# ChristophReich1996/Multi-StyleGAN

Measured on AMD Instinct MI355X. Metric: training images/sec (G+D step, 256^2, seq=3x2ch), higher is better.
Workload: dtype bf16

## Files before the change

### include/msg_hip.h

```cpp
#ifndef MSG_HIP_H
#define MSG_HIP_H

#ifdef __cplusplus
extern "C" {
#endif

enum { MSG_OK = 0, MSG_EINVAL = -1, MSG_EUNSUPPORTED = -2, MSG_ELAUNCH = -3 };
enum { MSG_F32 = 0, MSG_BF16 = 1, MSG_F16 = 2, MSG_F64 = 3, MSG_F32_SPLIT = 4 };

#define MSG_ABI_VERSION 5
int msg_abi_version(void);
const char* msg_build_arch(void);
const char* msg_strerror(int code);

int msg_upfirdn2d(const void* x, const float* fir, void* y, int dtype,
                  int major, int in_h, int in_w, int minor, int kh, int kw,
                  int up_x, int up_y, int down_x, int down_y,
                  int pad_x0, int pad_x1, int pad_y0, int pad_y1, void* stream);

int msg_upfirdn2d_pitched(const void* x, const float* fir, void* y, int dtype,
                          int major, int in_h, int in_w, int minor, int in_pitch, int kh, int kw,
                          int up_x, int up_y, int down_x, int down_y,
                          int pad_x0, int pad_x1, int pad_y0, int pad_y1, void* stream);

// ... 128 lines not shown
                         int B, int IH, int IW, int Cx, int Ck, int OH, int OW, int N, int ldy,
                         int kh, int kw, int stride, int pad, long long w_batch_stride,
                         const float* act_bias, const float* noise, const float* noise_weight,
                         int noise_batch, float alpha, float scale, void* stream);
int msg_conv2d_fprop_act_mask(const void* x, const void* w, void* y, int dtype,
                              int B, int IH, int IW, int Cx, int Ck, int OH, int OW, int N, int ldy,
                              int kh, int kw, int stride, int pad, long long w_batch_stride,
                              const float* act_bias, const float* noise, const float* noise_weight,
                              int noise_batch, float alpha, float scale, unsigned char* mask, void* stream);

int msg_conv2d_fprop_residual(const void* x, const void* w, void* y, int dtype,
                              int B, int IH, int IW, int Cx, int Ck, int OH, int OW, int N, int ldy,
                              int kh, int kw, int stride, int pad, long long w_batch_stride,
                              const void* residual, int res_ld, float gain, void* stream);

long long msg_conv2d_fprop_act_backward_workspace(int dtype, int B, int IH, int IW, int Cx, int Ck, int OH, int OW,
                                                  int N, int kh, int kw, long long w_batch_stride, int has_noise);
int msg_conv2d_fprop_act_backward(const void* x, const void* w, void* y, int dtype,
                                  int B, int IH, int IW, int Cx, int Ck, int OH, int OW, int N, int ldy,
                                  int kh, int kw, int stride, int pad, long long w_batch_stride,
                                  const void* residual, int res_ld,
                                  const unsigned char* sign_mask, int mask_tile_m, int mask_tile_n,
                                  const void* sign_map, int sign_ld, float alpha, float scale,
                                  float* grad_bias, const float* noise, int noise_batch, float* grad_noise_weight,
                                  float* ws, long long ws_floats, void* stream);

int msg_act_pointwise_head(const void* x, const float* bias, const float* w, float* y, int dtype,
                           long long npix, int C, float wscale, float alpha, float scale, void* stream);
long long msg_act_pointwise_head_backward_workspace(long long npix, int C);
int msg_act_pointwise_head_backward(const void* x, const float* bias, const float* w, const float* gy, void* gx,
// ... 43 lines not shown
```

### multi_stylegan_amd/conv_ops.py

```python
import math
import os
from typing import Optional, Tuple

import torch
from torch.autograd import Function

from . import _lib
from ._autograd import _derive


def _vec(dtype) -> int:
    return 8 if dtype == torch.bfloat16 else 4


def _round_up(n: int, m: int) -> int:
    return (n + m - 1) // m * m


def _padded_nhwc(b, c, h, w, dtype, device):
    cx = _round_up(c, _vec(dtype))
    buf = torch.empty((b, h, w, cx), dtype=dtype, device=device)
    if cx != c:
        buf[..., c:].zero_()
    return buf.permute(0, 3, 1, 2)[:, :c]
# ... 323 lines not shown
    def set(mode: str) -> None:
        fp32_contraction(mode).__enter__()


def _contraction_code(t: torch.Tensor, mode: Optional[str] = None) -> int:
    code = _lib.dtype_code(t)
    mode = FP32_CONTRACTION if mode is None else mode
    return _SPLIT_CODES[mode] if (code == _lib.MSG_F32 and mode != "exact") else code


_PLANS = {_lib.MSG_PLAN_REG: ("conv_fprop_reg", None), _lib.MSG_PLAN_DMA: ("conv_fprop_dma", None),
          _lib.MSG_PLAN_PP: ("conv_fprop_pp", None), _lib.MSG_PLAN_ROW3: ("conv_fprop_row3", 256),
          _lib.MSG_PLAN_ROW3N: ("conv_fprop_row3n", 128), _lib.MSG_PLAN_THIN: ("conv_fprop_thin", None)}
_PLAN_CACHE: dict = {}
_WGRAD_WS_CACHE: dict = {}


def _launch_fprop(x, wk, ck, bias, n, out_hw, kh, kw, stride, pad, in_up, pixel_shuffle, per_sample, c_real,
                  flops=None, act=None, residual=None, out=None, mode=None):
    dev = _lib.require_gpu(x, wk, bias)
    xv, cx = _nhwc_view(x)
    b, _, ih, iw = xv.shape
    oh, ow = out_hw
    if out is not None:
        y, ldy = _nhwc_view(out)
        if y is not out or pixel_shuffle or out.shape != (b, n, oh, ow) or out.dtype != x.dtype or n % _vec(x.dtype):
            raise _lib.MsgHipError(f"conv fprop: destination {tuple(out.shape)} / {out.stride()} for a {(b, n, oh, ow)} result")
    elif pixel_shuffle:
        y, ldy = _alloc_out(b, n // 4, 2 * oh, 2 * ow, x.dtype, dev)
    else:
# ... 8 lines not shown
        raise _lib.MsgHipError(f"conv fprop: weight image {tuple(wk.shape)} smaller than {n} x {kh * kw} x {ck}")
    wstride = wk.stride(0) if per_sample else 0
    if flops is None:
        flops = 2.0 * b * oh * ow * n * kh * kw * c_real / (in_up * in_up)
    key = "conv_fprop"
    if _lib.kernel_clock.enabled:
        plan = _lib.lib().msg_conv2d_fprop_plan(_lib.dtype_code(x), b, ih, iw, cx, ck, oh, ow, n, kh, kw, wstride)
        key = _PLANS[_lib.MSG_PLAN_REG if plan == _lib.MSG_PLAN_THIN and act is not None else plan][0]
        if x.dtype == torch.bfloat16 and bias is None and act is None and residual is None and \
                _lib.lib().msg_conv2d_fprop_upconv_eligible(b, ih, iw, cx, ck, oh, ow, n, kh, kw, stride, pad, in_up,
                                                           int(pixel_shuffle), wstride):
            key = "conv_fprop_upconv"
        if _CLOCK_SHAPES:
            key += f"|B{b} {ih}x{iw}->{oh}x{ow} {c_real}->{n} {kh}x{kw} s{stride} up{in_up}" \
                   f"{' ps' if pixel_shuffle else ''}{' per-sample' if per_sample else ''}|"
    with _lib.on_device(dev), _lib.kernel_clock.span((key, 'bf16' if x.dtype == torch.bfloat16 else 'f32'), flops):
        if residual is not None:
            assert bias is None and act is None and in_up == 1 and not pixel_shuffle
            rv, res_ld = _nhwc_view(residual[0])
            assert rv.shape == (b, n, oh, ow) and rv.dtype == x.dtype
            code = _lib.lib().msg_conv2d_fprop_residual(
                xv.data_ptr(), wk.data_ptr(), y.data_ptr(), _contraction_code(x, mode), b, ih, iw, cx, ck, oh, ow, n, ldy, kh, kw,
                stride, pad, wstride, rv.data_ptr(), res_ld, float(residual[1]), _lib.stream_of(dev))
        elif act is None:
            code = _lib.lib().msg_conv2d_fprop(
                xv.data_ptr(), wk.data_ptr(), _lib.ptr(bias), y.data_ptr(), _contraction_code(x, mode), b, ih, iw, cx, ck, oh,
                ow, n, ldy, kh, kw, stride, pad, in_up, int(pixel_shuffle), wstride, _lib.stream_of(dev))
        else:
            assert bias is None and in_up == 1 and not pixel_shuffle
            act_bias, noise, noise_w, alpha, scale = act[:5]
            _lib.require_gpu(x, act_bias, noise, noise_w)
            mask = None
            if len(act) > 5 and act[5] is not None and kh == 3 and stride == 1 and pad == 1:
                pkey = (x.dtype, b, ih, iw, cx, ck, oh, ow, n, kh, kw, wstride)
                mplan = _PLAN_CACHE.get(pkey)
                if mplan is None:
                    mplan = _PLAN_CACHE[pkey] = _lib.lib().msg_conv2d_fprop_plan(_lib.dtype_code(x), b, ih, iw, cx, ck, oh, ow,
                                                                                n, kh, kw, wstride)
                tile = _PLANS[mplan][1]
                if tile:
                    from .op_static.fused_act import sign_mask_for
                    mask = sign_mask_for(b, n, oh, ow, x.dtype, dev)
# ... 1320 lines not shown
```

### multi_stylegan_amd/csrc/conv_dispatch.h

```cpp
#pragma once
#include "msg_common.h"

struct ConvProblem {
    int dtype;
    int split;
    int B, IH, IW, Cx, Ck, OH, OW, N, ldy;
    int kh, kw, stride, pad, in_up, pixel_shuffle;
    long long w_batch_stride;

    bool per_sample() const { return w_batch_stride != 0; }
    int samples() const { return per_sample() ? B : 1; }
    long long mtot() const { return per_sample() ? (long long)OH * OW : (long long)B * OH * OW; }
    int esz() const { return dtype == MSG_BF16 ? 2 : 4; }
    long long x_bstride() const { return (long long)IH * IW * Cx; }
    long long y_bstride() const { return (pixel_shuffle ? 4ll : 1ll) * OH * OW * ldy; }
    long long x_bytes() const { return (long long)(per_sample() ? 1 : B) * IH * IW * Cx * esz(); }
    long long w_bytes() const { return (long long)N * kh * kw * Ck * esz(); }
    bool fits31() const { return x_bytes() < 0x7ffffff0ll && w_bytes() < 0x7ffffff0ll; }
};

enum ConvKernel {
    CONV_THIN_N, CONV_THIN_K,
    CONV_UPCONV,
    CONV_ROW3, CONV_ROW3N,
    CONV_PP,
    CONV_DMA, CONV_REG, CONV_REG_LEAN, CONV_REG_SPLIT
};

struct ConvPlan {
    ConvKernel kernel;
    int tile_m, tile_n;
    bool supported;
};

inline int conv_act_mode(const ActEpilogue* act) { return act ? act->enabled : 0; }

template <typename P>
inline void conv_fill_common(P& p, const ConvProblem& q, const ActEpilogue* act) {
    p.B = q.B; p.IH = q.IH; p.IW = q.IW; p.Cx = q.Cx; p.Ck = q.Ck; p.OH = q.OH; p.OW = q.OW; p.N = q.N; p.ldy = q.ldy;
    p.per_sample = q.per_sample();
    if (act) p.act = *act;
    p.x_bstride = q.x_bstride();
    p.w_bstride = q.w_batch_stride;
    p.y_bstride = q.y_bstride();
    p.Mtot = (int)q.mtot();
}
template <typename P>
// ... 32 lines not shown
```

### multi_stylegan_amd/csrc/conv_fprop.hip

```cpp
#include "conv_dispatch.h"
#include <stdlib.h>

typedef __bf16 bf16v8 __attribute__((ext_vector_type(8)));
typedef const __attribute__((address_space(1))) char* gptr_t;
typedef const __attribute__((address_space(1))) u32x4* gvec_t;
typedef __attribute__((address_space(3))) char* lds_t;

struct ConvParams {
    int B, IH, IW, Cx, Ck, OH, OW, N, ldy;
    int kh, kw, stride, pad, in_up, pixel_shuffle, per_sample;
    long long x_bstride, w_bstride, y_bstride;
    int Mtot, n_chunks, n_iters, m_tiles, n_tiles;
    ActEpilogue act;
};

constexpr int BM = 128, BN = 128, ROWB = 128;
constexpr int STAGE_BYTES = (BM + BN) * ROWB;
__device__ __attribute__((aligned(256))) unsigned int g_zero_page[16384];

__device__ __forceinline__ int swz(int row, int slot) { return row * ROWB + ((slot ^ ((row >> 1) & 7)) << 4); }

template <int SPLIT>
__device__ __forceinline__ void split_park(const u32x4& raw, char* dst) {
    uint2 pl[3];
#pragma unroll
    for (int h = 0; h < 2; ++h) {
        const float x0 = __uint_as_float(raw[2 * h]), x1 = __uint_as_float(raw[2 * h + 1]);
        const unsigned hp = (unsigned)f2bf(x0) | ((unsigned)f2bf(x1) << 16);
        const float r0 = x0 - __uint_as_float(hp << 16), r1 = x1 - __uint_as_float(hp & 0xffff0000u);
        const unsigned mp = (unsigned)f2bf(r0) | ((unsigned)f2bf(r1) << 16);
        (h ? pl[0].y : pl[0].x) = hp;
        (h ? pl[1].y : pl[1].x) = mp;
        if constexpr (SPLIT == 3) {
            const float q0 = r0 - __uint_as_float(mp << 16), q1 = r1 - __uint_as_float(mp & 0xffff0000u);
            (h ? pl[2].y : pl[2].x) = (unsigned)f2bf(q0) | ((unsigned)f2bf(q1) << 16);
        }
    }
#pragma unroll
    for (int p = 0; p < SPLIT; ++p) *reinterpret_cast<uint2*>(dst + p * 64) = pl[p];
}

template <typename T, bool DMA, int LEAN = 0, int SPLIT = 0>
__global__ __launch_bounds__(256, LEAN ? LEAN : 2) void conv_fprop_kernel(const T* __restrict__ x, const T* __restrict__ w,
                                                            T* __restrict__ y, const float* __restrict__ bias,
                                                            ConvParams p) {
    constexpr int VEC = 16 / sizeof(T);
    constexpr int BKE = ROWB / sizeof(T);
    static_assert(!LEAN || (!DMA && sizeof(T) == 2), "lean variant: bf16, register staging");
    static_assert(SPLIT == 0 || sizeof(T) == 4, "split-bf16 products are a mode of the fp32-storage kernel");
    static_assert(SPLIT == 0 || !DMA, "the split planes are written from the staging registers");
    constexpr int SROW = SPLIT ? SPLIT * 64 + 16 : ROWB;
    constexpr int STAGE = SPLIT ? (BM + BN) * SROW : STAGE_BYTES;
    constexpr bool ONE_STAGE = LEAN != 0 || SPLIT == 3;
    constexpr int SMEM_BYTES = ONE_STAGE ? (STAGE > 65536 || sizeof(T) == 2 ? STAGE : 65536) : 2 * STAGE;
    __shared__ __attribute__((aligned(16))) char smem[SMEM_BYTES];

    const int tid = threadIdx.x, lane = tid & 63, wid = tid >> 6;
    const int wm = wid >> 1, wn = wid & 1;
    const int lr = lane & 31, lh = lane >> 5;
    const unsigned L = xcd_remap(blockIdx.x, gridDim.x);
    const int n0 = (int)(L % p.n_tiles) * BN;
    const int m0 = (int)(L / p.n_tiles) * BM;
    const int bz = blockIdx.z;

    const int wid_u = __builtin_amdgcn_readfirstlane(wid);
    const int slot_phys = tid & 7;
    int row_of[4];
#pragma unroll
    for (int j = 0; j < 4; ++j) row_of[j] = DMA ? (wid * 32 + 8 * j + (lane >> 3)) : ((tid >> 3) + 32 * j);
    const int slot = DMA ? 0 : slot_phys;
    int a_ih0[4], a_iw0[4];
    long long a_boff[4];
    int a_slot[4];
    bool a_ok[4];
    const int ohw = p.OH * p.OW;
#pragma unroll
    for (int j = 0; j < 4; ++j) {
        const int m = m0 + row_of[j];
// ... 9 lines not shown
                     ((long long)a_ih0[j] * p.IW + a_iw0[j]) * p.Cx) * (long long)sizeof(T);
        a_slot[j] = slot_j;
    }
    const int taps = p.kh * p.kw;
    const gptr_t xbase = (gptr_t)x;
    const gptr_t zbase = (gptr_t)g_zero_page;
    const long long zoff = slot_phys * 16;
    gptr_t pa[4];
    gptr_t pb[4];
    {
        const gptr_t wb = (gptr_t)w + (p.per_sample ? (long long)bz * p.w_bstride : 0) * (long long)sizeof(T);
#pragma unroll
        for (int j = 0; j < 4; ++j) {
            const int n = n0 + row_of[j];
            const bool ok = n < p.N;
            pb[j] = (ok ? wb : zbase) + (ok ? ((long long)n * taps * p.Ck + a_slot[j] * VEC) * (long long)sizeof(T) : zoff);
            pa[j] = zbase;
        }
    }
    msg_desc_t d_x = {0, 0, 0, 0}, d_w = {0, 0, 0, 0};
    unsigned lds0 = 0;
    int va[4] = {MSG_DMA_OOB, MSG_DMA_OOB, MSG_DMA_OOB, MSG_DMA_OOB}, vb[4] = {MSG_DMA_OOB, MSG_DMA_OOB, MSG_DMA_OOB, MSG_DMA_OOB};
    if constexpr (DMA) {
        d_x = msg_make_desc((const char*)x + (p.per_sample ? (long long)bz * p.x_bstride * (long long)sizeof(T) : 0));
        d_w = msg_make_desc((const char*)w + (p.per_sample ? (long long)bz * p.w_bstride * (long long)sizeof(T) : 0));
        lds0 = (unsigned)(unsigned long long)(lds_t)smem;
#pragma unroll
        for (int j = 0; j < 4; ++j) {
            const int n = n0 + row_of[j];
            vb[j] = n < p.N ? (int)(((long long)n * taps * p.Ck + a_slot[j] * VEC) * (long long)sizeof(T)) : MSG_DMA_OOB;
        }
    }
    const bool ragged = (p.Cx % BKE) != 0;
    int ld_tap = -1, ld_chunk = p.n_chunks - 1;
    int kh_ = 0, kw_ = -1;
    int st_off[4];
#pragma unroll
    for (int j = 0; j < 4; ++j) st_off[j] = swz(row_of[j], a_slot[j]);

    f32x16 acc[2][2];
#pragma unroll
    for (int i = 0; i < 2; ++i)
#pragma unroll
        for (int j = 0; j < 2; ++j)
#pragma unroll
            for (int e = 0; e < 16; ++e) acc[i][j][e] = 0.f;

    u32x4 ra[4], rb[4];
    int dma_stage = 0;
    auto load_next = [&]() __attribute__((always_inline)) {
        if (++ld_chunk == p.n_chunks) {
            ld_chunk = 0;
            ++ld_tap;
            if (++kw_ == p.kw) { kw_ = 0; ++kh_; }
            if (p.in_up == 1) {
                const long long tap_off = ((long long)kh_ * p.IW + kw_) * p.Cx * (long long)sizeof(T);
#pragma unroll
                for (int j = 0; j < 4; ++j) {
                    const bool ok = a_ok[j] & ((unsigned)(a_ih0[j] + kh_) < (unsigned)p.IH) &
                                    ((unsigned)(a_iw0[j] + kw_) < (unsigned)p.IW);
                    pa[j] = (ok ? xbase : zbase) + (ok ? a_boff[j] + tap_off : zoff);
                    if constexpr (DMA) va[j] = ok ? (int)(a_boff[j] + tap_off) : MSG_DMA_OOB;
                }
            } else {
#pragma unroll
                for (int j = 0; j < 4; ++j) {
                    const int ih = a_ih0[j] + kh_, iw = a_iw0[j] + kw_;
                    bool ok = a_ok[j] & (ih >= 0) & (iw >= 0) & (ih % p.in_up == 0) & (iw % p.in_up == 0);
                    const int ihs = ih / p.in_up, iws = iw / p.in_up;
                    ok = ok & (ihs < p.IH) & (iws < p.IW);
                    const long long off = a_boff[j] + ((long long)(ihs - a_ih0[j]) * p.IW + (iws - a_iw0[j])) * p.Cx * (long long)sizeof(T);
                    pa[j] = (ok ? xbase : zbase) + (ok ? off : zoff);
                    if constexpr (DMA) va[j] = ok ? (int)off : MSG_DMA_OOB;
                }
            }
        }
#pragma unroll
        for (int j = 0; j < 4; ++j) {
            const bool c_bad = ragged && (ld_chunk * BKE + a_slot[j] * VEC + VEC > p.Cx);
            gptr_t a_addr = pa[j];
            if (c_bad) a_addr = zbase + zoff;
            if constexpr (DMA) {
                const unsigned la = lds0 + dma_stage * STAGE + (wid_u * 32 + 8 * j) * ROWB;
                msg_dma16(d_x, la, c_bad ? MSG_DMA_OOB : va[j], ld_chunk * ROWB);
                msg_dma16(d_w, la + BM * ROWB, vb[j], (ld_tap * p.n_chunks + ld_chunk) * ROWB);
            } else {
                ra[j] = *(gvec_t)a_addr;
// ... 83 lines not shown
                    fa[t] = *reinterpret_cast<const f32x4*>(sa + swz(wm * 64 + t * 32 + lr, 4 * lh + q));
                    fb[t] = *reinterpret_cast<const f32x4*>(sb + swz(wn * 64 + t * 32 + lr, 4 * lh + q));
                }
#pragma unroll
                for (int e = 0; e < 4; ++e)
#pragma unroll
                    for (int i = 0; i < 2; ++i)
#pragma unroll
                        for (int j = 0; j < 2; ++j)
                            acc[i][j] = __builtin_amdgcn_mfma_f32_32x32x2f32(fb[j][e], fa[i][e], acc[i][j], 0, 0, 0);
            }
        }
    };
    if constexpr (ONE_STAGE) {
        load_next();
        for (int it = 0; it < p.n_iters; ++it) {
            if (it) __syncthreads();
            park(0);
            if (it + 1 < p.n_iters) load_next();
            __syncthreads();
            mma_step(smem);
        }
    } else {
        if constexpr (DMA) {
            dma_stage = 0;
            load_next();
        } else {
            load_next();
            park(0);
            if (p.n_iters > 1) load_next();
        }
        for (int it = 0; it < p.n_iters; ++it) {
            if constexpr (DMA) asm volatile("s_waitcnt vmcnt(0)" ::: "memory");
            __syncthreads();
            if constexpr (DMA) {
                if (it + 1 < p.n_iters) { dma_stage = (it + 1) & 1; load_next(); }
            } else {
                if (it + 1 < p.n_iters) park((it + 1) & 1);
                if (it + 2 < p.n_iters) load_next();
            }
            mma_step(smem + (it & 1) * STAGE);
        }
    }
    if constexpr (DMA) asm volatile("s_waitcnt vmcnt(0)" ::: "memory");
    __syncthreads();

    constexpr int PITCH = 64 * sizeof(T);
    constexpr int UNITB = 4 * sizeof(T);
    char* ep = smem + wid * (64 * PITCH);
#pragma unroll
    for (int j = 0; j < 2; ++j)
#pragma unroll
        for (int g = 0; g < 4; ++g) {
            const int unit = 8 * j + 2 * g + lh;
            float bv[4] = {0.f, 0.f, 0.f, 0.f};
            if (bias) {
                const int nb = n0 + wn * 64 + 4 * unit;
#pragma unroll
                for (int e = 0; e < 4; ++e) bv[e] = nb + e < p.N ? bias[nb + e] : 0.f;
            }
#pragma unroll
// ... 79 lines not shown
#pragma unroll
        for (int pass = 0; pass < NPASS; ++pass)
            if (gp[pass] >= 0) *reinterpret_cast<u32x4*>(ybase + (long long)gp[pass] * p.ldy) = v[pass];
    } else if (n_ok) {
#pragma unroll
        for (int pass = 0; pass < NPASS; ++pass) {
            if (gp[pass] < 0) continue;
            T tmp[VEC];
            *reinterpret_cast<u32x4*>(tmp) = v[pass];
            T* dst = ybase + (long long)gp[pass] * p.ldy;
            for (int e = 0; e < lim; ++e) dst[e] = tmp[e];
        }
    }
}

static ConvPlan conv_generic_select(const ConvProblem& q) {
    const int n_iters = q.kh * q.kw * (q.Ck / (ROWB / q.esz()));
    static const int variant = msg_tunable("MSG_CONV_VARIANT", 0);
    const bool dma = q.fits31() && (variant == 1 || (variant == 0 && n_iters >= 8));
    static const int lean_max = msg_tunable("MSG_CONV_LEAN", 4);
    ConvPlan plan{CONV_REG, BM, BN, true};
    if (q.split) plan.kernel = CONV_REG_SPLIT;
    else if (dma) plan.kernel = CONV_DMA;
    else if (q.dtype == MSG_BF16 && n_iters <= lean_max) plan.kernel = CONV_REG_LEAN;
    const long long mtot = q.mtot(), blocks = ((mtot + BM - 1) / BM) * ((q.N + BN - 1) / BN);
    plan.supported = mtot < (1ll << 31) && blocks < (1ll << 31) &&
                     (long long)(n_iters + 1) * ROWB + 128 <= 65536;
    return plan;
}

static void conv_generic_launch(const ConvProblem& q, const ConvPlan& plan, const void* x, const void* w, const float* bias, void* y,
                                const ActEpilogue* act, void* stream) {
    ConvParams p{};
    conv_fill_common(p, q, act);
    conv_fill_taps(p, q);
    p.n_chunks = q.Ck / (ROWB / q.esz());
    p.n_iters = q.kh * q.kw * p.n_chunks;
    p.m_tiles = (int)((q.mtot() + BM - 1) / BM);
    p.n_tiles = (q.N + BN - 1) / BN;
    dim3 grid((unsigned)((long long)p.m_tiles * p.n_tiles), 1, q.samples());
#define GENERIC(T, ...) hipLaunchKernelGGL((conv_fprop_kernel<T, __VA_ARGS__>), grid, dim3(256), 0, (hipStream_t)stream, \
                                           (const T*)x, (const T*)w, (T*)y, bias, p)
    const bool bf16 = q.dtype == MSG_BF16;
    if (bf16 && plan.kernel == CONV_REG_LEAN) GENERIC(bf16_t, false, 3);
    else if (bf16 && plan.kernel == CONV_DMA) GENERIC(bf16_t, true);
    else if (bf16) GENERIC(bf16_t, false);
    else if (plan.kernel == CONV_REG_SPLIT) GENERIC(float, false, 0, 3);
    else if (plan.kernel == CONV_DMA) GENERIC(float, true);
    else GENERIC(float, false);
#undef GENERIC
}

ConvPlan conv_fprop_select(const ConvProblem& q, const ActEpilogue* act, bool has_bias) {
    ConvPlan plan;
    if (conv_thin_eligible(q, act, &plan)) return plan;
    if (conv_upconv_eligible(q, act, has_bias, &plan)) return plan;
    if (conv_row3_eligible(q, act, has_bias, &plan)) return plan;
    if (conv_pp_eligible(q, &plan)) return plan;
    return conv_generic_select(q);
// ... 12 lines not shown

extern "C" int msg_conv2d_fprop_plan(int dtype, int B, int IH, int IW, int Cx, int Ck, int OH, int OW, int N,
                                     int kh, int kw, long long w_batch_stride) {
    switch (conv_fprop_select(conv_query_problem(dtype, B, IH, IW, Cx, Ck, OH, OW, N, kh, kw, w_batch_stride), nullptr, false).kernel) {
        case CONV_THIN_N: case CONV_THIN_K: return MSG_PLAN_THIN;
        case CONV_ROW3: return MSG_PLAN_ROW3;
        case CONV_ROW3N: return MSG_PLAN_ROW3N;
        case CONV_PP: return MSG_PLAN_PP;
        case CONV_UPCONV: return MSG_PLAN_PP;
        case CONV_DMA: return MSG_PLAN_DMA;
        default: return MSG_PLAN_REG;
    }
}

static int conv2d_fprop_impl(const void* x, const void* w, const float* bias, void* y, const ConvProblem& q,
                             const ActEpilogue& act, void* stream, const ConvPlan* selected = nullptr);

extern "C" int msg_conv2d_fprop(const void* x, const void* w, const float* bias, void* y, int dtype,
                                int B, int IH, int IW, int Cx, int Ck, int OH, int OW, int N, int ldy,
                                int kh, int kw, int stride, int pad, int in_up, int pixel_shuffle,
                                long long w_batch_stride, void* stream) {
    ActEpilogue act{};
    return conv2d_fprop_impl(x, w, bias, y, conv_problem(dtype, B, IH, IW, Cx, Ck, OH, OW, N, ldy, kh, kw, stride, pad, in_up,
                                                         pixel_shuffle, w_batch_stride), act, stream);
}

static bool is_row3(const ConvPlan& plan) { return plan.kernel == CONV_ROW3 || plan.kernel == CONV_ROW3N; }

extern "C" int msg_conv2d_fprop_act_mask(const void* x, const void* w, void* y, int dtype,
                                         int B, int IH, int IW, int Cx, int Ck, int OH, int OW, int N, int ldy,
                                         int kh, int kw, int stride, int pad, long long w_batch_stride,
                                         const float* act_bias, const float* noise, const float* noise_weight,
                                         int noise_batch, float alpha, float scale, unsigned char* mask, void* stream) {
    if (noise && (!noise_weight || (noise_batch != 1 && noise_batch != B))) return MSG_EINVAL;
    const ConvProblem q = conv_problem(dtype, B, IH, IW, Cx, Ck, OH, OW, N, ldy, kh, kw, stride, pad, 1, 0, w_batch_stride);
    ActEpilogue act{act_bias, noise, noise_weight, noise_batch, 1, alpha, scale, nullptr, 0, 0.f, mask};
    if (!mask) return conv2d_fprop_impl(x, w, nullptr, y, q, act, stream);
    const ConvPlan plan = conv_fprop_select(q, &act, false);
    return is_row3(plan) ? conv2d_fprop_impl(x, w, nullptr, y, q, act, stream, &plan) : (int)MSG_EUNSUPPORTED;
}

extern "C" int msg_conv2d_fprop_act(const void* x, const void* w, void* y, int dtype,
                                    int B, int IH, int IW, int Cx, int Ck, int OH, int OW, int N, int ldy,
                                    int kh, int kw, int stride, int pad, long long w_batch_stride,
                                    const float* act_bias, const float* noise, const float* noise_weight,
                                    int noise_batch, float alpha, float scale, void* stream) {
    return msg_conv2d_fprop_act_mask(x, w, y, dtype, B, IH, IW, Cx, Ck, OH, OW, N, ldy, kh, kw, stride, pad, w_batch_stride,
                                     act_bias, noise, noise_weight, noise_batch, alpha, scale, nullptr, stream);
}

extern "C" int msg_conv2d_fprop_residual(const void* x, const void* w, void* y, int dtype,
                                         int B, int IH, int IW, int Cx, int Ck, int OH, int OW, int N, int ldy,
                                         int kh, int kw, int stride, int pad, long long w_batch_stride,
                                         const void* residual, int res_ld, float gain, void* stream) {
    if (!residual || res_ld < N || (((uintptr_t)residual) & 15u) || res_ld % (dtype == MSG_BF16 ? 8 : 4)) return MSG_EINVAL;
    ActEpilogue act{};
    act.enabled = 2; act.residual = residual; act.res_ld = res_ld; act.res_gain = gain;
    return conv2d_fprop_impl(x, w, nullptr, y, conv_problem(dtype, B, IH, IW, Cx, Ck, OH, OW, N, ldy, kh, kw, stride, pad, 1, 0,
                                                            w_batch_stride), act, stream);
}

static void act_backward_partials(const ConvProblem& q, const ConvPlan& plan, long long* rows, long long* entries) {
    *rows = *entries = 0;
    if (!is_row3(plan)) return;
    const long long tiles = (q.mtot() / plan.tile_m) * q.samples();
    *rows = tiles * 2;
    *entries = tiles * (q.N / plan.tile_n) * 4;
}

extern "C" long long msg_conv2d_fprop_act_backward_workspace(int dtype, int B, int IH, int IW, int Cx, int Ck, int OH, int OW,
                                                             int N, int kh, int kw, long long w_batch_stride, int has_noise) {
    const ConvProblem q = conv_query_problem(dtype, B, IH, IW, Cx, Ck, OH, OW, N, kh, kw, w_batch_stride);
    ActEpilogue act{};
    act.enabled = 3;
// ... 30 lines not shown
    if (has_noise && noise_batch != 1 && noise_batch != B) return MSG_EINVAL;
    const long long need_b = grad_bias ? rows * N : 0, need_n = has_noise ? entries : 0;
    if (need_b + need_n > 0 && (!ws || ws_floats < need_b + need_n)) return MSG_EINVAL;
    act.residual = residual; act.res_ld = res_ld; act.res_gain = 1.f;
    act.mask = const_cast<unsigned char*>(sign_mask); act.mask_tile_m = mask_tile_m; act.mask_tile_n = mask_tile_n;
    act.sign_src = sign_map; act.sign_ld = sign_ld;
    act.noise = has_noise ? noise : nullptr; act.noise_batch = noise_batch;
    act.part_b = grad_bias ? ws : nullptr;
    act.part_n = has_noise ? ws + need_b : nullptr;
    conv_row3_launch(q, plan, x, w, nullptr, y, &act, stream);
    if (MSG_CHECK_LAUNCH() != MSG_OK) return MSG_ELAUNCH;
    return msg_bias_act_reduce_launch(act.part_b, grad_bias, N, rows, act.part_n, grad_noise_weight, entries, stream);
}

static int conv2d_fprop_impl(const void* x, const void* w, const float* bias, void* y, const ConvProblem& q,
                             const ActEpilogue& act, void* stream, const ConvPlan* selected) {
    if (q.B == 0) return MSG_OK;
    if (!x || !w || !y || q.B < 0 || q.IH <= 0 || q.IW <= 0 || q.OH <= 0 || q.OW <= 0 || q.N <= 0 || q.kh <= 0 || q.kw <= 0 ||
        q.stride <= 0 || q.in_up <= 0 || q.Cx <= 0 || q.Ck <= 0 || q.ldy <= 0)
        return MSG_EINVAL;
    if (q.dtype != MSG_F32 && q.dtype != MSG_BF16) return MSG_EUNSUPPORTED;
    const int vec = 16 / q.esz(), bke = ROWB / q.esz();
    if (q.Ck % bke || q.Cx % vec || (((uintptr_t)x | (uintptr_t)w | (uintptr_t)y) & 15u)) return MSG_EUNSUPPORTED;
    if (q.ldy % vec || (q.pixel_shuffle && (q.N % 4 || (q.N / 4) % vec))) return MSG_EUNSUPPORTED;
    if (q.in_up > 1 && q.stride != 1) return MSG_EUNSUPPORTED;
    const ConvPlan plan = selected ? *selected : conv_fprop_select(q, &act, bias != nullptr);
    if (!plan.supported) return MSG_EUNSUPPORTED;
    switch (plan.kernel) {
        case CONV_THIN_N: case CONV_THIN_K: conv_thin_launch(q, plan, x, w, bias, y, &act, stream); break;
        case CONV_UPCONV: conv_upconv_launch(q, plan, x, w, y, stream); break;
        case CONV_ROW3: case CONV_ROW3N: conv_row3_launch(q, plan, x, w, bias, y, &act, stream); break;
        case CONV_PP: conv_pp_launch(q, plan, x, w, bias, y, &act, stream); break;
        case CONV_DMA: case CONV_REG: case CONV_REG_LEAN: case CONV_REG_SPLIT:
            conv_generic_launch(q, plan, x, w, bias, y, &act, stream); break;
    }
    return MSG_CHECK_LAUNCH();
}
```

Baseline: 155.0.

## Add split-K slicing with fp32 slab reduction for bf16 generic conv fprop

Adds a K-slice mode to the generic bf16 conv forward kernel. Each slice covers a contiguous range of tap/chunk iterations and writes fp32 partial sums to a workspace slab. A separate reduce kernel then sums the slices and applies bias, activation or residual epilogues. A cost model picks the slice count, so small-M, deep-K convolutions can fill more of the GPU. The cost is extra global memory traffic for the slabs, an extra launch, and workspace allocation from Python.

```diff
diff --git a/include/msg_hip.h b/include/msg_hip.h
--- a/include/msg_hip.h
+++ b/include/msg_hip.h
@@ -166,6 +166,24 @@
                               int kh, int kw, int stride, int pad, long long w_batch_stride,
                               const void* residual, int res_ld, float gain, void* stream);
 
+long long msg_conv2d_fprop_kslice_workspace(int dtype, int B, int IH, int IW, int Cx, int Ck, int OH, int OW, int N,
+                                            int ldy, int kh, int kw, int stride, int pad, int in_up, int pixel_shuffle,
+                                            long long w_batch_stride, int has_bias, int epilogue);
+int msg_conv2d_fprop_ws(const void* x, const void* w, const float* bias, void* y, int dtype,
+                        int B, int IH, int IW, int Cx, int Ck, int OH, int OW, int N, int ldy,
+                        int kh, int kw, int stride, int pad, int in_up, int pixel_shuffle,
+                        long long w_batch_stride, float* ws, long long ws_floats, void* stream);
+int msg_conv2d_fprop_act_ws(const void* x, const void* w, void* y, int dtype,
+                            int B, int IH, int IW, int Cx, int Ck, int OH, int OW, int N, int ldy,
+                            int kh, int kw, int stride, int pad, long long w_batch_stride,
+                            const float* act_bias, const float* noise, const float* noise_weight,
+                            int noise_batch, float alpha, float scale, float* ws, long long ws_floats, void* stream);
+int msg_conv2d_fprop_residual_ws(const void* x, const void* w, void* y, int dtype,
+                                 int B, int IH, int IW, int Cx, int Ck, int OH, int OW, int N, int ldy,
+                                 int kh, int kw, int stride, int pad, long long w_batch_stride,
+                                 const void* residual, int res_ld, float gain,
+                                 float* ws, long long ws_floats, void* stream);
+
 long long msg_conv2d_fprop_act_backward_workspace(int dtype, int B, int IH, int IW, int Cx, int Ck, int OH, int OW,
                                                   int N, int kh, int kw, long long w_batch_stride, int has_noise);
 int msg_conv2d_fprop_act_backward(const void* x, const void* w, void* y, int dtype,
diff --git a/multi_stylegan_amd/conv_ops.py b/multi_stylegan_amd/conv_ops.py
--- a/multi_stylegan_amd/conv_ops.py
+++ b/multi_stylegan_amd/conv_ops.py
@@ -361,6 +361,8 @@
           _lib.MSG_PLAN_ROW3N: ("conv_fprop_row3n", 128), _lib.MSG_PLAN_THIN: ("conv_fprop_thin", None)}
 _PLAN_CACHE: dict = {}
 _WGRAD_WS_CACHE: dict = {}
+_KSLICE_WS_CACHE: dict = {}
+K_SLICES = bool(int(os.environ.get("MSG_CONV_K_SLICES", "1")))
 
 
 def _launch_fprop(x, wk, ck, bias, n, out_hw, kh, kw, stride, pad, in_up, pixel_shuffle, per_sample, c_real,
@@ -399,18 +401,47 @@
         if _CLOCK_SHAPES:
             key += f"|B{b} {ih}x{iw}->{oh}x{ow} {c_real}->{n} {kh}x{kw} s{stride} up{in_up}" \
                    f"{' ps' if pixel_shuffle else ''}{' per-sample' if per_sample else ''}|"
+    need = 0
+    if K_SLICES and x.dtype == torch.bfloat16:
+        skey = (b, ih, iw, cx, ck, oh, ow, n, ldy, kh, kw, stride, pad, in_up, pixel_shuffle, wstride, bias is None,
+                residual is None, act is None)
+        need = _KSLICE_WS_CACHE.get(skey)
+        if need is None:
+            need = _KSLICE_WS_CACHE[skey] = _lib.lib().msg_conv2d_fprop_kslice_workspace(
+                _lib.MSG_BF16, b, ih, iw, cx, ck, oh, ow, n, ldy, kh, kw, stride, pad, in_up, int(pixel_shuffle), wstride,
+                int(bias is not None), 2 if residual is not None else 0 if act is None else 1)
     with _lib.on_device(dev), _lib.kernel_clock.span((key, 'bf16' if x.dtype == torch.bfloat16 else 'f32'), flops):
         if residual is not None:
             assert bias is None and act is None and in_up == 1 and not pixel_shuffle
             rv, res_ld = _nhwc_view(residual[0])
             assert rv.shape == (b, n, oh, ow) and rv.dtype == x.dtype
-            code = _lib.lib().msg_conv2d_fprop_residual(
-                xv.data_ptr(), wk.data_ptr(), y.data_ptr(), _contraction_code(x, mode), b, ih, iw, cx, ck, oh, ow, n, ldy, kh, kw,
-                stride, pad, wstride, rv.data_ptr(), res_ld, float(residual[1]), _lib.stream_of(dev))
+            if need:
+                code = _lib.lib().msg_conv2d_fprop_residual_ws(
+                    xv.data_ptr(), wk.data_ptr(), y.data_ptr(), _lib.MSG_BF16, b, ih, iw, cx, ck, oh, ow, n, ldy, kh, kw,
+                    stride, pad, wstride, rv.data_ptr(), res_ld, float(residual[1]), _lib.scratch_ptr(need, dev), need,
+                    _lib.stream_of(dev))
+            else:
+                code = _lib.lib().msg_conv2d_fprop_residual(
+                    xv.data_ptr(), wk.data_ptr(), y.data_ptr(), _contraction_code(x, mode), b, ih, iw, cx, ck, oh, ow, n, ldy, kh, kw,
+                    stride, pad, wstride, rv.data_ptr(), res_ld, float(residual[1]), _lib.stream_of(dev))
+        elif act is None and need:
+            code = _lib.lib().msg_conv2d_fprop_ws(
+                xv.data_ptr(), wk.data_ptr(), _lib.ptr(bias), y.data_ptr(), _lib.MSG_BF16, b, ih, iw, cx, ck, oh,
+                ow, n, ldy, kh, kw, stride, pad, in_up, int(pixel_shuffle), wstride, _lib.scratch_ptr(need, dev), need,
+                _lib.stream_of(dev))
         elif act is None:
             code = _lib.lib().msg_conv2d_fprop(
                 xv.data_ptr(), wk.data_ptr(), _lib.ptr(bias), y.data_ptr(), _contraction_code(x, mode), b, ih, iw, cx, ck, oh,
                 ow, n, ldy, kh, kw, stride, pad, in_up, int(pixel_shuffle), wstride, _lib.stream_of(dev))
+        elif need:
+            assert bias is None and in_up == 1 and not pixel_shuffle
+            act_bias, noise, noise_w, alpha, scale = act[:5]
+            _lib.require_gpu(x, act_bias, noise, noise_w)
+            code = _lib.lib().msg_conv2d_fprop_act_ws(
+                xv.data_ptr(), wk.data_ptr(), y.data_ptr(), _lib.MSG_BF16, b, ih, iw, cx, ck, oh, ow, n, ldy, kh, kw,
+                stride, pad, wstride, _lib.ptr(act_bias), _lib.ptr(noise), _lib.ptr(noise_w),
+                1 if noise is None else noise.shape[0], float(alpha), float(scale), _lib.scratch_ptr(need, dev), need,
+                _lib.stream_of(dev))
         else:
             assert bias is None and in_up == 1 and not pixel_shuffle
             act_bias, noise, noise_w, alpha, scale = act[:5]
diff --git a/multi_stylegan_amd/csrc/conv_dispatch.h b/multi_stylegan_amd/csrc/conv_dispatch.h
--- a/multi_stylegan_amd/csrc/conv_dispatch.h
+++ b/multi_stylegan_amd/csrc/conv_dispatch.h
@@ -31,6 +31,7 @@
     ConvKernel kernel;
     int tile_m, tile_n;
     bool supported;
+    int k_slices = 1;
 };
 
 inline int conv_act_mode(const ActEpilogue* act) { return act ? act->enabled : 0; }
diff --git a/multi_stylegan_amd/csrc/conv_fprop.hip b/multi_stylegan_amd/csrc/conv_fprop.hip
--- a/multi_stylegan_amd/csrc/conv_fprop.hip
+++ b/multi_stylegan_amd/csrc/conv_fprop.hip
@@ -1,5 +1,6 @@
 #include "conv_dispatch.h"
 #include <stdlib.h>
+#include <algorithm>
 
 typedef __bf16 bf16v8 __attribute__((ext_vector_type(8)));
 typedef const __attribute__((address_space(1))) char* gptr_t;
@@ -11,6 +12,8 @@
     int kh, kw, stride, pad, in_up, pixel_shuffle, per_sample;
     long long x_bstride, w_bstride, y_bstride;
     int Mtot, n_chunks, n_iters, m_tiles, n_tiles;
+    int k_slices;
+    float* slabs;
     ActEpilogue act;
 };
 
@@ -40,7 +43,7 @@
     for (int p = 0; p < SPLIT; ++p) *reinterpret_cast<uint2*>(dst + p * 64) = pl[p];
 }
 
-template <typename T, bool DMA, int LEAN = 0, int SPLIT = 0>
+template <typename T, bool DMA, int LEAN = 0, int SPLIT = 0, bool KSLICE = false>
 __global__ __launch_bounds__(256, LEAN ? LEAN : 2) void conv_fprop_kernel(const T* __restrict__ x, const T* __restrict__ w,
                                                             T* __restrict__ y, const float* __restrict__ bias,
                                                             ConvParams p) {
@@ -49,6 +52,7 @@
     static_assert(!LEAN || (!DMA && sizeof(T) == 2), "lean variant: bf16, register staging");
     static_assert(SPLIT == 0 || sizeof(T) == 4, "split-bf16 products are a mode of the fp32-storage kernel");
     static_assert(SPLIT == 0 || !DMA, "the split planes are written from the staging registers");
+    static_assert(!KSLICE || (sizeof(T) == 2 && !LEAN), "K slices: the bf16 DMA / register-staged instantiations");
     constexpr int SROW = SPLIT ? SPLIT * 64 + 16 : ROWB;
     constexpr int STAGE = SPLIT ? (BM + BN) * SROW : STAGE_BYTES;
     constexpr bool ONE_STAGE = LEAN != 0 || SPLIT == 3;
@@ -62,6 +66,10 @@
     const int n0 = (int)(L % p.n_tiles) * BN;
     const int m0 = (int)(L / p.n_tiles) * BM;
     const int bz = blockIdx.z;
+    const int slice = KSLICE ? (int)blockIdx.y : 0;
+    const int it_per = KSLICE ? (p.n_iters + p.k_slices - 1) / p.k_slices : p.n_iters;
+    const int it0 = slice * it_per;
+    const int n_it = KSLICE ? min(it_per, p.n_iters - it0) : p.n_iters;
 
     const int wid_u = __builtin_amdgcn_readfirstlane(wid);
     const int slot_phys = tid & 7;
@@ -101,7 +109,7 @@
         for (int j = 0; j < 4; ++j) {
             const int n = n0 + row_of[j];
             const bool ok = n < p.N;
-            pb[j] = (ok ? wb : zbase) + (ok ? ((long long)n * taps * p.Ck + a_slot[j] * VEC) * (long long)sizeof(T) : zoff);
+            pb[j] = (ok ? wb : zbase) + (ok ? ((long long)n * taps * p.Ck + a_slot[j] * VEC) * (long long)sizeof(T) + (long long)it0 * ROWB : zoff);
             pa[j] = zbase;
         }
     }
@@ -121,6 +129,14 @@
     const bool ragged = (p.Cx % BKE) != 0;
     int ld_tap = -1, ld_chunk = p.n_chunks - 1;
     int kh_ = 0, kw_ = -1;
+    int skip = 0;
+    if constexpr (KSLICE) {
+        const int tap0 = it0 / p.n_chunks;
+        skip = it0 - tap0 * p.n_chunks;
+        ld_tap = tap0 - 1;
+        kh_ = tap0 / p.kw;
+        kw_ = tap0 - kh_ * p.kw - 1;
+    }
     int st_off[4];
 #pragma unroll
     for (int j = 0; j < 4; ++j) st_off[j] = swz(row_of[j], a_slot[j]);
@@ -140,13 +156,15 @@
             ld_chunk = 0;
             ++ld_tap;
             if (++kw_ == p.kw) { kw_ = 0; ++kh_; }
+            long long skip_off = 0;
+            if constexpr (KSLICE) { ld_chunk = skip; skip_off = (long long)skip * ROWB; skip = 0; }
             if (p.in_up == 1) {
                 const long long tap_off = ((long long)kh_ * p.IW + kw_) * p.Cx * (long long)sizeof(T);
 #pragma unroll
                 for (int j = 0; j < 4; ++j) {
                     const bool ok = a_ok[j] & ((unsigned)(a_ih0[j] + kh_) < (unsigned)p.IH) &
                                     ((unsigned)(a_iw0[j] + kw_) < (unsigned)p.IW);
-                    pa[j] = (ok ? xbase : zbase) + (ok ? a_boff[j] + tap_off : zoff);
+                    pa[j] = (ok ? xbase : zbase) + (ok ? a_boff[j] + tap_off + skip_off : zoff);
                     if constexpr (DMA) va[j] = ok ? (int)(a_boff[j] + tap_off) : MSG_DMA_OOB;
                 }
             } else {
@@ -157,7 +175,7 @@
                     const int ihs = ih / p.in_up, iws = iw / p.in_up;
                     ok = ok & (ihs < p.IH) & (iws < p.IW);
                     const long long off = a_boff[j] + ((long long)(ihs - a_ih0[j]) * p.IW + (iws - a_iw0[j])) * p.Cx * (long long)sizeof(T);
-                    pa[j] = (ok ? xbase : zbase) + (ok ? off : zoff);
+                    pa[j] = (ok ? xbase : zbase) + (ok ? off + skip_off : zoff);
                     if constexpr (DMA) va[j] = ok ? (int)off : MSG_DMA_OOB;
                 }
             }
@@ -271,10 +289,10 @@
     };
     if constexpr (ONE_STAGE) {
         load_next();
-        for (int it = 0; it < p.n_iters; ++it) {
+        for (int it = 0; it < n_it; ++it) {
             if (it) __syncthreads();
             park(0);
-            if (it + 1 < p.n_iters) load_next();
+            if (it + 1 < n_it) load_next();
             __syncthreads();
             mma_step(smem);
         }
@@ -285,16 +303,16 @@
         } else {
             load_next();
             park(0);
-            if (p.n_iters > 1) load_next();
-        }
-        for (int it = 0; it < p.n_iters; ++it) {
+            if (n_it > 1) load_next();
+        }
+        for (int it = 0; it < n_it; ++it) {
             if constexpr (DMA) asm volatile("s_waitcnt vmcnt(0)" ::: "memory");
             __syncthreads();
             if constexpr (DMA) {
-                if (it + 1 < p.n_iters) { dma_stage = (it + 1) & 1; load_next(); }
+                if (it + 1 < n_it) { dma_stage = (it + 1) & 1; load_next(); }
             } else {
-                if (it + 1 < p.n_iters) park((it + 1) & 1);
-                if (it + 2 < p.n_iters) load_next();
+                if (it + 1 < n_it) park((it + 1) & 1);
+                if (it + 2 < n_it) load_next();
             }
             mma_step(smem + (it & 1) * STAGE);
         }
@@ -302,6 +320,22 @@
     if constexpr (DMA) asm volatile("s_waitcnt vmcnt(0)" ::: "memory");
     __syncthreads();
 
+    if constexpr (KSLICE) {
+        const int npad = p.n_tiles * BN;
+        float* slab = p.slabs + ((long long)bz * p.k_slices + slice) * p.Mtot * npad + n0 + wn * 64 + 4 * lh;
+#pragma unroll
+        for (int i = 0; i < 2; ++i) {
+            const int m = m0 + wm * 64 + 32 * i + lr;
+            if (m >= p.Mtot) continue;
+#pragma unroll
+            for (int j = 0; j < 2; ++j)
+#pragma unroll
+                for (int g = 0; g < 4; ++g)
+                    *reinterpret_cast<f32x4*>(slab + (long long)m * npad + 32 * j + 8 * g) =
+                        f32x4{acc[i][j][4 * g + 0], acc[i][j][4 * g + 1], acc[i][j][4 * g + 2], acc[i][j][4 * g + 3]};
+        }
+        return;
+    }
     constexpr int PITCH = 64 * sizeof(T);
     constexpr int UNITB = 4 * sizeof(T);
     char* ep = smem + wid * (64 * PITCH);
@@ -411,6 +445,89 @@
     }
 }
 
+__global__ __launch_bounds__(256) void conv_kslice_reduce_kernel(bf16_t* __restrict__ y, const float* __restrict__ bias, ConvParams p) {
+    constexpr int VEC = 8;
+    const int vpr = (p.N + VEC - 1) / VEC;
+    const long long idx = (long long)blockIdx.x * 256 + threadIdx.x;
+    if (idx >= (long long)p.Mtot * vpr) return;
+    const int m = (int)(idx / vpr), n = (int)(idx - (long long)m * vpr) * VEC, bz = blockIdx.z;
+    const int npad = p.n_tiles * BN;
+    const long long slab = (long long)p.Mtot * npad;
+    const float* src = p.slabs + (long long)bz * p.k_slices * slab + (long long)m * npad + n;
+    f32x4 lo = *reinterpret_cast<const f32x4*>(src), hi = *reinterpret_cast<const f32x4*>(src + 4);
+    for (int sl = 1; sl < p.k_slices; ++sl) {
+        lo += *reinterpret_cast<const f32x4*>(src + sl * slab);
+        hi += *reinterpret_cast<const f32x4*>(src + sl * slab + 4);
+    }
+    u32x4 v;
+#pragma unroll
+    for (int e = 0; e < 4; ++e) {
+        const float s0 = e < 2 ? lo[2 * e] : hi[2 * e - 4], s1 = e < 2 ? lo[2 * e + 1] : hi[2 * e - 3];
+        const float b0 = (bias && n + 2 * e < p.N) ? bias[n + 2 * e] : 0.f, b1 = (bias && n + 2 * e + 1 < p.N) ? bias[n + 2 * e + 1] : 0.f;
+        v[e] = (unsigned)f2bf(s0 + b0) | ((unsigned)f2bf(s1 + b1) << 16);
+    }
+    const int ohw = p.OH * p.OW;
+    const int b = p.per_sample ? bz : m / ohw;
+    const int pix = p.per_sample ? m : m - b * ohw;
+    const int oh = pix / p.OW, ow = pix - oh * p.OW;
+    int nn = n, q = 0;
+    if (p.pixel_shuffle) { const int oc = p.N >> 2; q = n / oc; nn = n - q * oc; }
+    const int lim = p.pixel_shuffle ? (p.N >> 2) - nn : p.N - n;
+    const long long gp = p.pixel_shuffle ? ((long long)(b * 2 * p.OH + 2 * oh + (q >> 1)) * (2 * p.OW) + 2 * ow + (q & 1))
+                                         : (long long)b * ohw + pix;
+    if (p.act.enabled == 1) {
+        float a_bias[VEC];
+#pragma unroll
+        for (int e = 0; e < VEC; ++e) a_bias[e] = (p.act.bias && n + e < p.N) ? p.act.bias[n + e] : 0.f;
+        const float a_noise = p.act.noise ? p.act.noise_w[0] * p.act.noise[(long long)(p.act.noise_batch == 1 ? 0 : b) * ohw + pix] : 0.f;
+        v = act_epilogue_apply<bf16_t>(v, a_bias, a_noise, p.act.alpha, p.act.scale);
+    } else if (p.act.enabled == 2) {
+        const u32x4 r = *reinterpret_cast<const u32x4*>(reinterpret_cast<const bf16_t*>(p.act.residual) + gp * p.act.res_ld + nn);
+        v = residual_epilogue_apply<bf16_t>(v, r, p.act.res_gain);
+    }
+    bf16_t* dst = y + gp * p.ldy + nn;
+    if (lim >= VEC) {
+        *reinterpret_cast<u32x4*>(dst) = v;
+    } else {
+        bf16_t tmp[VEC];
+        *reinterpret_cast<u32x4*>(tmp) = v;
+        for (int e = 0; e < lim; ++e) dst[e] = tmp[e];
+    }
+}
+
+static int conv_generic_slices(const ConvProblem& q, ConvKernel kernel, int n_iters) {
+    constexpr int SLOTS = 512, KS_MIN_STEPS = 6, KS_MAX = 16;
+    constexpr double KS_STEP1 = 750, KS_STEP2 = 1000, KS_FIXED = 6000, KS_BYTES_PER_NS = 3000, KS_GAIN = 0.85;
+    if (q.dtype != MSG_BF16 || (kernel != CONV_DMA && kernel != CONV_REG)) return 1;
+    const long long mtot = q.mtot(), n_tiles = (q.N + BN - 1) / BN;
+    const long long wgs = ((mtot + BM - 1) / BM) * n_tiles * q.samples();
+    const int most = (int)std::min<long long>(KS_MAX, std::min<long long>(n_iters, 65535));
+    auto whole = [&](int s) { return (s - 1) * ((n_iters + s - 1) / s) < n_iters; };
+    const int forced = msg_tunable("MSG_CONV_KSLICES", 0);
+    if (forced > 0) {
+        int s = std::min(forced, most);
+        while (!whole(s)) --s;
+        return s;
+    }
+    if (wgs >= SLOTS) return 1;
+    auto model = [&](int s) {
+        const int steps = (n_iters + s - 1) / s;
+        const double slab_bytes = 4.0 * q.samples() * s * mtot * n_tiles * BN;
+        return steps * (wgs * s <= SLOTS / 2 ? KS_STEP1 : KS_STEP2) + (s > 1 ? KS_FIXED + 2 * slab_bytes / KS_BYTES_PER_NS : 0.0);
+    };
+    int best = 1;
+    double t_best = model(1) * KS_GAIN;
+    for (int s = 2; s <= most && wgs * s <= SLOTS && n_iters / s >= KS_MIN_STEPS; ++s) {
+        if (!whole(s)) continue;
+        const double t = model(s);
+        if (t < t_best) { best = s; t_best = t; }
+    }
+    return best;
+}
+static long long conv_generic_slab_floats(const ConvProblem& q, const ConvPlan& plan) {
+    return plan.k_slices > 1 ? (long long)q.samples() * plan.k_slices * q.mtot() * ((q.N + BN - 1) / BN) * BN : 0;
+}
+
 static ConvPlan conv_generic_select(const ConvProblem& q) {
     const int n_iters = q.kh * q.kw * (q.Ck / (ROWB / q.esz()));
     static const int variant = msg_tunable("MSG_CONV_VARIANT", 0);
@@ -423,11 +540,12 @@
     const long long mtot = q.mtot(), blocks = ((mtot + BM - 1) / BM) * ((q.N + BN - 1) / BN);
     plan.supported = mtot < (1ll << 31) && blocks < (1ll << 31) &&
                      (long long)(n_iters + 1) * ROWB + 128 <= 65536;
+    if (plan.supported) plan.k_slices = conv_generic_slices(q, plan.kernel, n_iters);
     return plan;
 }
 
 static void conv_generic_launch(const ConvProblem& q, const ConvPlan& plan, const void* x, const void* w, const float* bias, void* y,
-                                const ActEpilogue* act, void* stream) {
+                                const ActEpilogue* act, float* ws, void* stream) {
     ConvParams p{};
     conv_fill_common(p, q, act);
     conv_fill_taps(p, q);
@@ -435,11 +553,19 @@
     p.n_iters = q.kh * q.kw * p.n_chunks;
     p.m_tiles = (int)((q.mtot() + BM - 1) / BM);
     p.n_tiles = (q.N + BN - 1) / BN;
-    dim3 grid((unsigned)((long long)p.m_tiles * p.n_tiles), 1, q.samples());
+    p.k_slices = ws ? plan.k_slices : 1;
+    p.slabs = ws;
+    dim3 grid((unsigned)((long long)p.m_tiles * p.n_tiles), p.k_slices, q.samples());
 #define GENERIC(T, ...) hipLaunchKernelGGL((conv_fprop_kernel<T, __VA_ARGS__>), grid, dim3(256), 0, (hipStream_t)stream, \
                                            (const T*)x, (const T*)w, (T*)y, bias, p)
     const bool bf16 = q.dtype == MSG_BF16;
-    if (bf16 && plan.kernel == CONV_REG_LEAN) GENERIC(bf16_t, false, 3);
+    if (p.k_slices > 1) {
+        if (plan.kernel == CONV_DMA) GENERIC(bf16_t, true, 0, 0, true);
+        else GENERIC(bf16_t, false, 0, 0, true);
+        const long long vecs = (long long)p.Mtot * ((p.N + 7) / 8);
+        hipLaunchKernelGGL(conv_kslice_reduce_kernel, dim3((unsigned)((vecs + 255) / 256), 1, q.samples()), dim3(256), 0,
+                           (hipStream_t)stream, (bf16_t*)y, bias, p);
+    } else if (bf16 && plan.kernel == CONV_REG_LEAN) GENERIC(bf16_t, false, 3);
     else if (bf16 && plan.kernel == CONV_DMA) GENERIC(bf16_t, true);
     else if (bf16) GENERIC(bf16_t, false);
     else if (plan.kernel == CONV_REG_SPLIT) GENERIC(float, false, 0, 3);
@@ -482,18 +608,50 @@
 }
 
 static int conv2d_fprop_impl(const void* x, const void* w, const float* bias, void* y, const ConvProblem& q,
-                             const ActEpilogue& act, void* stream, const ConvPlan* selected = nullptr);
+                             const ActEpilogue& act, void* stream, const ConvPlan* selected = nullptr, float* ws = nullptr,
+                             long long ws_floats = 0);
+
+extern "C" long long msg_conv2d_fprop_kslice_workspace(int dtype, int B, int IH, int IW, int Cx, int Ck, int OH, int OW, int N,
+                                                       int ldy, int kh, int kw, int stride, int pad, int in_up, int pixel_shuffle,
+                                                       long long w_batch_stride, int has_bias, int epilogue) {
+    if (B <= 0 || IH <= 0 || IW <= 0 || OH <= 0 || OW <= 0 || N <= 0 || kh <= 0 || kw <= 0 || Cx <= 0 || Ck <= 0) return 0;
+    if (dtype != MSG_BF16 || Ck % (ROWB / 2) || epilogue < 0 || epilogue > 2) return 0;
+    const ConvProblem q = conv_problem(dtype, B, IH, IW, Cx, Ck, OH, OW, N, ldy, kh, kw, stride, pad, in_up, pixel_shuffle, w_batch_stride);
+    ActEpilogue act{};
+    act.enabled = epilogue;
+    const ConvPlan plan = conv_fprop_select(q, &act, has_bias != 0);
+    return (plan.supported && (plan.kernel == CONV_DMA || plan.kernel == CONV_REG)) ? conv_generic_slab_floats(q, plan) : 0;
+}
+
+extern "C" int msg_conv2d_fprop_ws(const void* x, const void* w, const float* bias, void* y, int dtype,
+                                   int B, int IH, int IW, int Cx, int Ck, int OH, int OW, int N, int ldy,
+                                   int kh, int kw, int stride, int pad, int in_up, int pixel_shuffle,
+                                   long long w_batch_stride, float* ws, long long ws_floats, void* stream) {
+    ActEpilogue act{};
+    return conv2d_fprop_impl(x, w, bias, y, conv_problem(dtype, B, IH, IW, Cx, Ck, OH, OW, N, ldy, kh, kw, stride, pad, in_up,
+                                                         pixel_shuffle, w_batch_stride), act, stream, nullptr, ws, ws_floats);
+}
 
 extern "C" int msg_conv2d_fprop(const void* x, const void* w, const float* bias, void* y, int dtype,
                                 int B, int IH, int IW, int Cx, int Ck, int OH, int OW, int N, int ldy,
                                 int kh, int kw, int stride, int pad, int in_up, int pixel_shuffle,
                                 long long w_batch_stride, void* stream) {
-    ActEpilogue act{};
-    return conv2d_fprop_impl(x, w, bias, y, conv_problem(dtype, B, IH, IW, Cx, Ck, OH, OW, N, ldy, kh, kw, stride, pad, in_up,
-                                                         pixel_shuffle, w_batch_stride), act, stream);
+    return msg_conv2d_fprop_ws(x, w, bias, y, dtype, B, IH, IW, Cx, Ck, OH, OW, N, ldy, kh, kw, stride, pad, in_up, pixel_shuffle,
+                               w_batch_stride, nullptr, 0, stream);
 }
 
 static bool is_row3(const ConvPlan& plan) { return plan.kernel == CONV_ROW3 || plan.kernel == CONV_ROW3N; }
+
+extern "C" int msg_conv2d_fprop_act_ws(const void* x, const void* w, void* y, int dtype,
+                                       int B, int IH, int IW, int Cx, int Ck, int OH, int OW, int N, int ldy,
+                                       int kh, int kw, int stride, int pad, long long w_batch_stride,
+                                       const float* act_bias, const float* noise, const float* noise_weight,
+                                       int noise_batch, float alpha, float scale, float* ws, long long ws_floats, void* stream) {
+    if (noise && (!noise_weight || (noise_batch != 1 && noise_batch != B))) return MSG_EINVAL;
+    ActEpilogue act{act_bias, noise, noise_weight, noise_batch, 1, alpha, scale, nullptr, 0, 0.f, nullptr};
+    return conv2d_fprop_impl(x, w, nullptr, y, conv_problem(dtype, B, IH, IW, Cx, Ck, OH, OW, N, ldy, kh, kw, stride, pad, 1, 0,
+                                                            w_batch_stride), act, stream, nullptr, ws, ws_floats);
+}
 
 extern "C" int msg_conv2d_fprop_act_mask(const void* x, const void* w, void* y, int dtype,
                                          int B, int IH, int IW, int Cx, int Ck, int OH, int OW, int N, int ldy,
@@ -503,7 +661,8 @@
     if (noise && (!noise_weight || (noise_batch != 1 && noise_batch != B))) return MSG_EINVAL;
     const ConvProblem q = conv_problem(dtype, B, IH, IW, Cx, Ck, OH, OW, N, ldy, kh, kw, stride, pad, 1, 0, w_batch_stride);
     ActEpilogue act{act_bias, noise, noise_weight, noise_batch, 1, alpha, scale, nullptr, 0, 0.f, mask};
-    if (!mask) return conv2d_fprop_impl(x, w, nullptr, y, q, act, stream);
+    if (!mask) return msg_conv2d_fprop_act_ws(x, w, y, dtype, B, IH, IW, Cx, Ck, OH, OW, N, ldy, kh, kw, stride, pad, w_batch_stride,
+                                              act_bias, noise, noise_weight, noise_batch, alpha, scale, nullptr, 0, stream);
     const ConvPlan plan = conv_fprop_select(q, &act, false);
     return is_row3(plan) ? conv2d_fprop_impl(x, w, nullptr, y, q, act, stream, &plan) : (int)MSG_EUNSUPPORTED;
 }
@@ -521,11 +680,20 @@
                                          int B, int IH, int IW, int Cx, int Ck, int OH, int OW, int N, int ldy,
                                          int kh, int kw, int stride, int pad, long long w_batch_stride,
                                          const void* residual, int res_ld, float gain, void* stream) {
+    return msg_conv2d_fprop_residual_ws(x, w, y, dtype, B, IH, IW, Cx, Ck, OH, OW, N, ldy, kh, kw, stride, pad, w_batch_stride,
+                                        residual, res_ld, gain, nullptr, 0, stream);
+}
+
+extern "C" int msg_conv2d_fprop_residual_ws(const void* x, const void* w, void* y, int dtype,
+                                            int B, int IH, int IW, int Cx, int Ck, int OH, int OW, int N, int ldy,
+                                            int kh, int kw, int stride, int pad, long long w_batch_stride,
+                                            const void* residual, int res_ld, float gain,
+                                            float* ws, long long ws_floats, void* stream) {
     if (!residual || res_ld < N || (((uintptr_t)residual) & 15u) || res_ld % (dtype == MSG_BF16 ? 8 : 4)) return MSG_EINVAL;
     ActEpilogue act{};
     act.enabled = 2; act.residual = residual; act.res_ld = res_ld; act.res_gain = gain;
     return conv2d_fprop_impl(x, w, nullptr, y, conv_problem(dtype, B, IH, IW, Cx, Ck, OH, OW, N, ldy, kh, kw, stride, pad, 1, 0,
-                                                            w_batch_stride), act, stream);
+                                                            w_batch_stride), act, stream, nullptr, ws, ws_floats);
 }
 
 static void act_backward_partials(const ConvProblem& q, const ConvPlan& plan, long long* rows, long long* entries) {
@@ -586,7 +754,7 @@
 }
 
 static int conv2d_fprop_impl(const void* x, const void* w, const float* bias, void* y, const ConvProblem& q,
-                             const ActEpilogue& act, void* stream, const ConvPlan* selected) {
+                             const ActEpilogue& act, void* stream, const ConvPlan* selected, float* ws, long long ws_floats) {
     if (q.B == 0) return MSG_OK;
     if (!x || !w || !y || q.B < 0 || q.IH <= 0 || q.IW <= 0 || q.OH <= 0 || q.OW <= 0 || q.N <= 0 || q.kh <= 0 || q.kw <= 0 ||
         q.stride <= 0 || q.in_up <= 0 || q.Cx <= 0 || q.Ck <= 0 || q.ldy <= 0)
@@ -604,7 +772,9 @@
         case CONV_ROW3: case CONV_ROW3N: conv_row3_launch(q, plan, x, w, bias, y, &act, stream); break;
         case CONV_PP: conv_pp_launch(q, plan, x, w, bias, y, &act, stream); break;
         case CONV_DMA: case CONV_REG: case CONV_REG_LEAN: case CONV_REG_SPLIT:
-            conv_generic_launch(q, plan, x, w, bias, y, &act, stream); break;
+            if (plan.k_slices > 1 && ws && (((uintptr_t)ws) & 15u)) return MSG_EINVAL;
+            if (plan.k_slices > 1 && ws && ws_floats < conv_generic_slab_floats(q, plan)) return MSG_EINVAL;
+            conv_generic_launch(q, plan, x, w, bias, y, &act, plan.k_slices > 1 ? ws : nullptr, stream); break;
     }
     return MSG_CHECK_LAUNCH();
 }
```

Measured after the change: 155.8 (median of 2 runs). No clear change (+0.5%).
